# majidsina/rlmd

Hardware: NVIDIA B200
Metric: investor-steps/sec (leverage sweep) (higher is better)
Workload: dtype 2-bit codes, int32 counts, f64 log-wealth, f32 wealth

## Files before the change

include/rlmd_b200.h:

```cpp
#ifndef RLMD_B200_H
#define RLMD_B200_H

#include <stdint.h>

#ifdef __cplusplus
extern "C" {
#endif

#define B200_OK 0
#define B200_EINVAL (-1)
#define B200_ECUDA (-2)
#define B200_ELIMIT (-3)

#define B200_MAX_PEERS 8

const char* b200_last_error(void);
int b200_version(void);
int b200_device_info(int32_t* sm_count, int32_t* cc_major, int32_t* cc_minor);

enum {
  B200_LEV_DISCRETE = 0,
  B200_LEV_GBM = 1
};
enum {
// ... 13 lines not shown
  int64_t ld_outcomes;
  int64_t investor_offset;
  int64_t ld_out;
  uint64_t seed;
  int32_t horizon;
  int32_t n_grid;
  int32_t n_outcomes;
  int32_t kind;
  int32_t source;
  int32_t mode;
  float value_0;
  float log_mean;
  float sigma;
  int32_t variant;
  uint32_t thresholds[B200_MAX_OUTCOMES];
  int32_t outcome_bits;
  int32_t flags;
} b200_lev_desc;

#define B200_LEV_FLAG_FINAL_ONLY 1
#define B200_LEV_FLAG_STATE_OUT 2
#define B200_LEV_FLAG_BESIDE_SWEEP 4
#define B200_LEV_FLAG_RADIX_SELECT 8

int b200_lev_sweep(const b200_lev_desc* desc, const void* outcomes,
                   const float* factors_host, float* data_T, double* log_w,
                   int32_t* counts, void* stream);

int b200_lev_chunk(const b200_lev_desc* desc, const void* outcomes,
                   const float* factors_host, int32_t t_begin, int32_t t_end,
                   void* state, float* dump, void* stream);

int b200_lev_draw(const b200_lev_desc* desc, void* out, void* stream);

int b200_lev_from_counts(const b200_lev_desc* desc, const int32_t* counts,
                         const float* factors_host, float* data_T, double* log_w,
                         void* stream);

int b200_lev_pack(const uint8_t* codes, int64_t n_investors, int32_t horizon,
                  int64_t ld_codes, uint8_t* packed, int64_t ld_packed, void* stream);
int b200_lev_pack_bits(const uint8_t* codes, int64_t n_investors, int32_t horizon,
                       int64_t ld_codes, uint8_t* packed, int64_t ld_packed, int32_t bits,
                       void* stream);

typedef struct b200_tally_plan {
  int64_t rows_cap;
// ... 230 lines not shown
```

rlmd_b200/_lib.py:

```python
import ctypes as C
import os

_HERE = os.path.dirname(os.path.abspath(__file__))
LIB_PATH = os.path.join(_HERE, "librlmd_b200.so")

B200_OK, B200_EINVAL, B200_ECUDA, B200_ELIMIT = 0, -1, -2, -3
LEV_DISCRETE, LEV_GBM = 0, 1
SRC_STREAM, SRC_PHILOX = 0, 1
MODE_CHAIN, MODE_LOG = 1, 2
MAX_GRID, MAX_OUTCOMES = 64, 4


class LevDesc(C.Structure):
    _fields_ = [
        ("n_investors", C.c_int64),
        ("ld_outcomes", C.c_int64),
        ("investor_offset", C.c_int64),
        ("ld_out", C.c_int64),
        ("seed", C.c_uint64),
        ("horizon", C.c_int32),
        ("n_grid", C.c_int32),
        ("n_outcomes", C.c_int32),
        ("kind", C.c_int32),
        ("source", C.c_int32),
        ("mode", C.c_int32),
        ("value_0", C.c_float),
        ("log_mean", C.c_float),
        ("sigma", C.c_float),
        ("variant", C.c_int32),
        ("thresholds", C.c_uint32 * MAX_OUTCOMES),
        ("outcome_bits", C.c_int32),
        ("flags", C.c_int32),
    ]


LEV_FLAG_FINAL_ONLY, LEV_FLAG_STATE_OUT, LEV_FLAG_BESIDE_SWEEP, LEV_FLAG_RADIX_SELECT = 1, 2, 4, 8
MAX_PEERS = 8


class PeerSet(C.Structure):
    _fields_ = [
        ("workspace", C.c_void_p * MAX_PEERS),
        ("flags", C.c_void_p * MAX_PEERS),
        ("stage", C.c_void_p * MAX_PEERS),
        ("stage_rows", C.c_int64),
        ("world", C.c_int32),
        ("rank", C.c_int32),
        ("epoch", C.c_uint32),
        ("reserved", C.c_uint32),
    ]


class TallyPlan(C.Structure):
    _fields_ = [
        ("rows_cap", C.c_int64),
        ("bins_cap", C.c_int64),
        ("grid_cap", C.c_int32),
        ("world", C.c_int32),
    ]
# ... 219 lines not shown
```

rlmd_b200/csrc/common.cu:

```cuda
#include "common.cuh"

#include <cstring>

namespace b200 {

static thread_local char g_err[512] = "";

int set_error(int code, const char* fmt, ...) {
  va_list ap;
  va_start(ap, fmt);
  vsnprintf(g_err, sizeof(g_err), fmt, ap);
  va_end(ap);
  return code;
}

int check_cuda(cudaError_t e, const char* what) {
  if (e == cudaSuccess) return 0;
  return set_error(B200_ECUDA, "%s: %s", what, cudaGetErrorString(e));
}

int sm_count() {
  static int cached[64] = {0};
  int dev = 0;
  if (cudaGetDevice(&dev) != cudaSuccess || dev < 0 || dev >= 64) { cudaGetLastError(); return 148; }
  if (cached[dev] == 0) {
    int n = 0;
    if (cudaDeviceGetAttribute(&n, cudaDevAttrMultiProcessorCount, dev) != cudaSuccess || n <= 0) {
      cudaGetLastError();
      n = 148;
    }
    cached[dev] = n;
  }
  return cached[dev];
}

__global__ void __launch_bounds__(256)
exchange_pack_kernel(const long long* __restrict__ ws, int64_t words, int64_t rows, int64_t io, int64_t ic,
                     int64_t d_o, int64_t dc, double* __restrict__ staging) {
  const int64_t per = ic + dc, total = rows * per;
  for (int64_t i = (int64_t)blockIdx.x * blockDim.x + threadIdx.x; i < total; i += (int64_t)gridDim.x * blockDim.x) {
    const int64_t r = i / per, k = i - r * per;
// ... 61 lines not shown
```

rlmd_b200/csrc/common.cuh:

```cuda
#pragma once

#include <cuda_runtime.h>
#include <stdint.h>

#include <cstdarg>
#include <cstdio>

#include "../../include/rlmd_b200.h"

namespace b200 {

int set_error(int code, const char* fmt, ...);
int check_cuda(cudaError_t e, const char* what);

#define B200_CUDA(expr)                                   \
  do {                                                    \
    int _rc = ::b200::check_cuda((expr), #expr);          \
    if (_rc != 0) return _rc;                             \
  } while (0)

#define B200_REQUIRE(cond, ...)                                     \
  do {                                                              \
    if (!(cond)) return ::b200::set_error(B200_EINVAL, __VA_ARGS__); \
  } while (0)

int sm_count();

struct Philox4 {
  uint32_t x, y, z, w;
};

__host__ __device__ __forceinline__ uint32_t mulhi32(uint32_t a, uint32_t b) {
#ifdef __CUDA_ARCH__
  return __umulhi(a, b);
#else
  return (uint32_t)(((uint64_t)a * (uint64_t)b) >> 32);
#endif
}

__host__ __device__ __forceinline__ Philox4 philox4x32_10(uint32_t c0, uint32_t c1, uint32_t c2,
                                                           uint32_t c3, uint32_t k0, uint32_t k1) {
  const uint32_t M0 = 0xD2511F53u, M1 = 0xCD9E8D57u;
  const uint32_t W0 = 0x9E3779B9u, W1 = 0xBB67AE85u;
#pragma unroll
  for (int r = 0; r < 10; ++r) {
    uint32_t hi0 = mulhi32(M0, c0), lo0 = M0 * c0;
    uint32_t hi1 = mulhi32(M1, c2), lo1 = M1 * c2;
    uint32_t n0 = hi1 ^ c1 ^ k0;
    uint32_t n2 = hi0 ^ c3 ^ k1;
// ... 160 lines not shown
```

rlmd_b200/csrc/lev_sweep.cu:

```cuda
#include <cstdlib>

#include "lev_kernels.cuh"
#include "tally.cuh"

namespace b200 {

struct LogFactorTable {
  double lm[B200_MAX_OUTCOMES][B200_MAX_GRID];
};
struct LevGrid {
  float lev[B200_MAX_GRID];
};

static int64_t out_ld(const b200_lev_desc& d) { return d.ld_out > 0 ? d.ld_out : d.n_investors; }

template <int K>
__global__ void __launch_bounds__(128)
draw_discrete_kernel(const __grid_constant__ Thresholds th, uint64_t seed, int64_t investor_offset, int32_t H,
                     int64_t N, int64_t ld, uint8_t* __restrict__ out) {
  const int nblk = (H + 3) >> 2;
  const int64_t idx = (int64_t)blockIdx.x * blockDim.x + threadIdx.x;
  if (idx >= N * nblk) return;
  const int64_t row = idx / nblk;
  const int j = (int)(idx - row * nblk);
// ... 206 lines not shown
}

constexpr int PACKED_U = 6;

template <int BITS>
__device__ __forceinline__ uint32_t word_mask(int valid) {
  constexpr int PER = 32 / BITS;
  const int v = min(max(valid, 0), PER);
  return v >= PER ? 0xffffffffu : ((1u << (BITS * v)) - 1u);
}
template <int BITS>
__device__ __forceinline__ uint4 last_vector_mask(int valid) {
  constexpr int PER = 32 / BITS;
  return make_uint4(word_mask<BITS>(valid), word_mask<BITS>(valid - PER), word_mask<BITS>(valid - 2 * PER),
                    word_mask<BITS>(valid - 3 * PER));
}

template <int K, bool TALLY, int BITS = 2>
__global__ void __launch_bounds__(COUNT_WARPS * 32, 4)
log_discrete_packed_kernel(const uint8_t* __restrict__ outcomes, int64_t ldb, int32_t H, int64_t N, int32_t G,
                           const __grid_constant__ LogFactorTable lf, double logV0, float* __restrict__ data_T,
                           double* __restrict__ log_w, int32_t* __restrict__ counts, int64_t ldT, const TallyDev tally,
                           int32_t task_rows) {
  const int lane = threadIdx.x & 31;
  const int64_t warp_global = (int64_t)blockIdx.x * COUNT_WARPS + (threadIdx.x >> 5);
  const int64_t nwarps = (int64_t)gridDim.x * COUNT_WARPS;
  constexpr int PER_BYTE = 8 / BITS;
  const int nbytes = (H + PER_BYTE - 1) / PER_BYTE;
  const int full = H / PER_BYTE;
  const int nvec = (nbytes + 15) >> 4;
  const bool vec_rows = (ldb & 15) == 0 && ldb >= (int64_t)nvec * 16;
  const int iters = (nvec + 32 * PACKED_U - 1) / (32 * PACKED_U);
  const int rem = nvec - (iters - 1) * 32 * PACKED_U;
  const int tail_slots = (rem + 31) >> 5;
  const int tail_lanes = rem - (tail_slots - 1) * 32;
  const bool in_tail = lane < tail_lanes;
  const uint4 wm = lane == tail_lanes - 1 ? last_vector_mask<BITS>(H - (128 / BITS) * (nvec - 1))
                                          : make_uint4(~0u, ~0u, ~0u, ~0u);
  auto count_byte = [&](int t, uint32_t& s1, uint32_t& s2, uint32_t& s3, const uint8_t* __restrict__ p) {
    uint32_t c = p[t];
    if (t >= full) c &= (1u << (BITS * (H % PER_BYTE))) - 1u;
    if (BITS == 1) { s1 += __popc(c); return; }
    s1 += __popc(c & 0x55u);
    if (K >= 3) s2 += __popc((c >> 1) & 0x55u);
    if (K >= 4) s3 += __popc(c & (c >> 1) & 0x55u);
  };
// ... 36 lines not shown
        }
      } else {
        const uintptr_t addr = (uintptr_t)p;
        int head = (int)((16 - (addr & 15)) & 15);
        if (head > full) head = full;
        const int body = (full - head) >> 4;
        const int tail0 = head + (body << 4);
        for (int t = lane; t < head; t += 32) count_byte(t, s1, s2, s3, p);
        const uint4* __restrict__ q = reinterpret_cast<const uint4*>(p + head);
        for (int i = lane; i < body; i += 32) {
          const uint4 a = __ldcs(q + i);
          count_pair<K, BITS>(a.x, a.y, s1, s2, s3); count_pair<K, BITS>(a.z, a.w, s1, s2, s3);
        }
        for (int t = tail0 + lane; t < nbytes; t += 32) count_byte(t, s1, s2, s3, p);
      }
#pragma unroll
      for (int o = 16; o > 0; o >>= 1) {
        s1 += __shfl_xor_sync(0xffffffffu, s1, o);
        if (K >= 3) s2 += __shfl_xor_sync(0xffffffffu, s2, o);
        if (K >= 4) s3 += __shfl_xor_sync(0xffffffffu, s3, o);
      }
      if (lane == r) { m1 = s1; m2 = s2; m3 = s3; }
    }
    if (lane < nr) {
      const int64_t row = row0 + lane;
      int n[4];
      if (K == 2) { n[1] = (int)m1; n[0] = H - n[1]; n[2] = n[3] = 0; }
      else if (K == 3) { n[1] = (int)m1; n[2] = (int)m2; n[0] = H - n[1] - n[2]; n[3] = 0; }
      else { n[3] = (int)m3; n[1] = (int)(m1 - m3); n[2] = (int)(m2 - m3); n[0] = H - n[1] - n[2] - n[3]; }
      if (counts != nullptr) {
#pragma unroll
        for (int k = 0; k < K; ++k) counts[row * K + k] = n[k];
      }
      if (TALLY) {
        tally_insert(tally, tally_key(n[1], n[2], n[3]), 1u);
        continue;
      }
      double nd[K];
#pragma unroll
      for (int k = 0; k < K; ++k) nd[k] = (double)n[k];
      for (int g = 0; g < G; ++g) {
        double lw = logV0;
#pragma unroll
        for (int k = 0; k < K; ++k)
          if (n[k] > 0) lw += nd[k] * lf.lm[k][g];
        if (log_w != nullptr) log_w[(int64_t)g * ldT + row] = lw;
// ... 348 lines not shown
      }
      lf.lm[k][g] = v;
    }
  return 0;
}

static int run_log_discrete(const b200_lev_desc& d, const uint8_t* outcomes, const float* factors_host,
                            float* data_T, double* log_w, int32_t* counts, const TallyDev& tally, cudaStream_t st) {
  LogFactorTable lf;
  if (factors_host != nullptr) {
    if (int rc = make_log_table(d, factors_host, lf)) return rc;
  } else {
    memset(&lf, 0, sizeof(lf));
  }
  const double logV0 = log((double)d.value_0);
  const int64_t N = d.n_investors;
  static const int task_rows = [] { const char* e = getenv("B200_PACKED_TASK_ROWS"); int v = e ? atoi(e) : 32;
                                    return v < 1 ? 1 : v > 32 ? 32 : v; }();
  const bool packed = d.outcome_bits == 2 || d.outcome_bits == 1;
  const int64_t warps = packed ? (N + task_rows - 1) / task_rows : N;
  int64_t blocks = (warps + COUNT_WARPS - 1) / COUNT_WARPS;
  const int64_t cap = packed ? (int64_t)0x7fffffff : (int64_t)sm_count() * 8;
  if (blocks > cap) blocks = cap;
#define B200_LOG_LAUNCH(KERNEL, ...)                                                                                     \
  KERNEL<__VA_ARGS__><<<(unsigned)blocks, COUNT_WARPS * 32, 0, st>>>(outcomes, d.ld_outcomes, d.horizon, N, d.n_grid, lf, \
                                                                     logV0, data_T, log_w, counts, out_ld(d), tally B200_EXTRA)
  if (d.outcome_bits == 1) {
#define B200_EXTRA , task_rows
    if (tally.keys != nullptr) B200_LOG_LAUNCH(log_discrete_packed_kernel, 2, true, 1);
    else B200_LOG_LAUNCH(log_discrete_packed_kernel, 2, false, 1);
#undef B200_EXTRA
  } else if (d.outcome_bits == 2) {
#define B200_EXTRA , task_rows
    if (tally.keys != nullptr) {
      switch (d.n_outcomes) {
        case 2: B200_LOG_LAUNCH(log_discrete_packed_kernel, 2, true); break;
        case 3: B200_LOG_LAUNCH(log_discrete_packed_kernel, 3, true); break;
        default: B200_LOG_LAUNCH(log_discrete_packed_kernel, 4, true); break;
      }
    } else {
      switch (d.n_outcomes) {
        case 2: B200_LOG_LAUNCH(log_discrete_packed_kernel, 2, false); break;
        case 3: B200_LOG_LAUNCH(log_discrete_packed_kernel, 3, false); break;
        default: B200_LOG_LAUNCH(log_discrete_packed_kernel, 4, false); break;
      }
    }
#undef B200_EXTRA
#define B200_EXTRA
  } else {
    switch (d.n_outcomes) {
      case 2: B200_LOG_LAUNCH(log_discrete_stream_kernel, 2); break;
      case 3: B200_LOG_LAUNCH(log_discrete_stream_kernel, 3); break;
      default: B200_LOG_LAUNCH(log_discrete_stream_kernel, 4); break;
    }
  }
#undef B200_LOG_LAUNCH
#undef B200_EXTRA
  return check_cuda(cudaGetLastError(), "log_discrete_stream launch");
}

static int run_log_gbm(const b200_lev_desc& d, const float* x, const float* lev_host, float* data_T, double* log_w,
                       cudaStream_t st) {
  LevGrid lv;
  for (int g = 0; g < B200_MAX_GRID; ++g) lv.lev[g] = g < d.n_grid ? lev_host[g] : 0.f;
  const double logV0 = log((double)d.value_0);
  const int64_t N = d.n_investors;
  const bool saturate = (d.flags & B200_LEV_FLAG_FINAL_ONLY) == 0;
  const int64_t state_n = (d.flags & B200_LEV_FLAG_STATE_OUT) ? N : 0;
// ... 360 lines not shown
```

rlmd_b200/csrc/tally.cu:

```cuda
#include <cooperative_groups.h>

#include <algorithm>
#include <cstdlib>
#include <cstring>

#include "tally.cuh"

namespace b200 {

struct BinEntry {
  unsigned long long key, count;
};
static_assert(sizeof(BinEntry) == 16, "one 16-byte vector per bin");

constexpr int MERGE_CHUNK = 2048;
constexpr int EX_FLAG_BYTES = 128;

struct LogTable {
  double lm[B200_MAX_OUTCOMES][B200_MAX_GRID];
};

struct TallyLayout {
  long long* header;
  unsigned long long* keysA; uint32_t* countsA; uint64_t capA;
// ... 99 lines not shown
    const uint32_t m = __reduce_max_sync(0xffffffffu, b[q]);
    if ((threadIdx.x & 31) == 0 && m != 0u) atomicMax(s + q, m);
  }
  __syncthreads();
  if (threadIdx.x < 4 && s[threadIdx.x] != 0u)
    atomicMax(reinterpret_cast<unsigned long long*>(dst) + threadIdx.x, (unsigned long long)s[threadIdx.x]);
}

constexpr int COMPACT_PER = 8;
constexpr int COMPACT_CHUNK = 256 * COMPACT_PER;

template <bool MULTI>
__global__ void __launch_bounds__(256)
tally_compact_kernel(TallyDev t, unsigned long long* __restrict__ ukeys, uint32_t* __restrict__ ucnt,
                     int64_t out_cap, const __grid_constant__ PeerView P) {
  __shared__ BinEntry stage[COMPACT_CHUNK];
  __shared__ int n_s;
  __shared__ long long base_s;
  __shared__ uint32_t box_s[4];
  uint32_t box[4] = {0, 0, 0, 0};
  const uint64_t cap = t.mask + 1;
  const uint64_t base = (uint64_t)blockIdx.x * COMPACT_CHUNK;
  if (threadIdx.x == 0) n_s = 0;
  __syncthreads();
  unsigned long long key[COMPACT_PER];
  uint32_t cnt[COMPACT_PER];
#pragma unroll
  for (int u = 0; u < COMPACT_PER; ++u) {
    const uint64_t i = base + (uint64_t)u * 256 + threadIdx.x;
    key[u] = i < cap ? __ldcg(t.keys + i) : TALLY_EMPTY;
    cnt[u] = i < cap ? __ldcg(t.counts + i) : 0u;
  }
#pragma unroll
  for (int u = 0; u < COMPACT_PER; ++u) {
    if (key[u] == TALLY_EMPTY) continue;
    const uint64_t i = base + (uint64_t)u * 256 + threadIdx.x;
    t.keys[i] = TALLY_EMPTY;
    t.counts[i] = 0;
    if (!MULTI) box_add(box, key[u]);
    const int p = atomicAdd(&n_s, 1);
    stage[p].key = key[u];
    stage[p].count = cnt[u];
  }
  __syncthreads();
  const int n = n_s;
  if (!MULTI && n > 0) box_flush(box, t.header + TH_BOX_ACC, box_s);
// ... 311 lines not shown
    for (int q = 0; q < N; ++q) {
      const double x = lane < (int)(blockDim.x >> 5) ? scratch[q * 32 + lane] : 0.0;
      v[q] = warp_sum(x);
    }
  }
}

template <int NK>
__global__ void __launch_bounds__(SEL_THREADS)
tally_select_kernel(long long* __restrict__ header, const unsigned long long* __restrict__ ukeys,
                    const uint32_t* __restrict__ ucnt, float* __restrict__ wbuf, int64_t ldw, int32_t H,
                    const __grid_constant__ LogTable lf, double logV0, int64_t n_total, int64_t top,
                    double* __restrict__ stats, int32_t SEL_CACHE ,
                    int32_t force_radix) {
  namespace cg = cooperative_groups;
  cg::cluster_group cluster = cg::this_cluster();
  const int C = (int)cluster.num_blocks(), r = (int)cluster.block_rank();
  __shared__ SelShared sh;
  extern __shared__ __align__(16) uint8_t dyn[];
  float* cw = reinterpret_cast<float*>(dyn);
  uint32_t* cc = reinterpret_cast<uint32_t*>(dyn) + SEL_CACHE;
  uint16_t* cb = reinterpret_cast<uint16_t*>(cc + SEL_CACHE);
  SelShared* L = cluster.map_shared_rank(&sh, 0);

  const int g = blockIdx.x / C;
  const long long B = header[TH_NBINS];
  const long long n = n_total, K = top;
  const double qnan = __longlong_as_double(0x7ff8000000000000LL);
  double* s = stats + (int64_t)g * 12;
  if (header[TH_TIMEOUT] != 0 || header[TH_OVERFLOW] != 0) {
    if (r == 0 && threadIdx.x < 12) s[threadIdx.x] = qnan;
    return;
  }
  const int tid = threadIdx.x, lane = threadIdx.x & 31;
#ifdef B200_TALLY_DEBUG
  int stamp_i = 0;
#define STAMP() do { if (r == 0 && tid == 0 && (g == 0 || g == (int)(gridDim.x / C) - 1)) { header[TH_DEBUG + (g == 0 ? 0 : 24) + stamp_i++] = clock64(); } } while (0)
#else
#define STAMP() do {} while (0)
#endif
  STAMP();
  const long long per = (((B + C - 1) / C) + 3) & ~3LL;
  const long long lo = min(B, (long long)r * per), hi = min(B, lo + per);
  const int m = (int)(hi - lo);
  float* __restrict__ w = wbuf + (int64_t)g * ldw + lo;
  const uint32_t* __restrict__ cnt = ucnt + lo;
// ... 464 lines not shown
      d0 += sh.part_d[q][0]; d1 += sh.part_d[q][1]; d2 += sh.part_d[q][2];
      d3 += sh.part_d[q][3]; d4 += sh.part_d[q][4]; d5 += sh.part_d[q][5];
    }
    const double thr = (double)key_float(thr_key);
    const double dt = thr - mean_t, da = thr - mean_j;
    const double tt = (double)sh.res_i[6], ta = (double)sh.res_i[7];
    const double abs_top = d0 + (tt > 0 ? tt * fabs(dt) : 0.0);
    const double sq_top = d1 + (tt > 0 ? tt * dt * dt : 0.0);
    const double abs_adj = d2 + (ta > 0 ? ta * fabs(da) : 0.0);
    const double sq_adj = d3 + (ta > 0 ? ta * da * da : 0.0);
    s[0] = mean_a; s[1] = mean_t; s[2] = mean_j;
    s[3] = d4 / (double)n; s[4] = abs_top / (double)K; s[5] = abs_adj / (double)(n - K);
    s[6] = sqrt(d5 / (double)n); s[7] = sqrt(sq_top / (double)K); s[8] = sqrt(sq_adj / (double)(n - K));
    s[9] = (double)key_float(key_j[0]); s[10] = (double)key_float(key_j[2]); s[11] = (double)key_float(key_j[3]);
    const long long size[3] = {n, K, n - K};
    const double single[3] = {qnan, thr, (double)key_float(key_j[3])};
    for (int j = 0; j < 3; ++j) {
      if (sh.res_i[j]) { s[0 + j] = size[j] == 1 ? single[j] : qnan; s[3 + j] = qnan; s[6 + j] = qnan; }
      if (sh.res_i[3 + j]) s[9 + j] = qnan;
    }
  }
}

static void select_shape(int& cluster, int& cache) {
  static int c = [] {
    const char* e = getenv("B200_SELECT_CLUSTER");
    int x = e ? atoi(e) : 6;
    return x < 1 ? 1 : x > SEL_MAX_CLUSTER ? SEL_MAX_CLUSTER : x;
  }();
  static int k = [] {
    const char* e = getenv("B200_SELECT_CACHE");
    int x = e ? atoi(e) : 16384;
    return x < 0 ? 0 : x > 20480 ? 20480 : x;
  }();
  cluster = c;
  cache = k;
}

template <int K>
static int launch_select_k(int n_grid, long long* header, const unsigned long long* ukeys, const uint32_t* ucnt,
                           float* wbuf, int64_t ldw, int32_t H, const LogTable& lf, double logV0, int64_t n_total,
                           int64_t top, double* stats, bool beside_sweep, bool force_radix, cudaStream_t st) {
  static bool attr_set[64] = {false};
  int dev = 0;
  B200_CUDA(cudaGetDevice(&dev));
  int C = 1, cache = 0;
  select_shape(C, cache);
  static const bool forced = getenv("B200_SELECT_CLUSTER") != nullptr;
  if (beside_sweep && !forced) C = 2;
  const size_t dyn = (size_t)cache * 10;
  if (dev < 64 && !attr_set[dev]) {
    B200_CUDA(cudaFuncSetAttribute(tally_select_kernel<K>, cudaFuncAttributeMaxDynamicSharedMemorySize, (int)dyn));
    if (C > 8) B200_CUDA(cudaFuncSetAttribute(tally_select_kernel<K>, cudaFuncAttributeNonPortableClusterSizeAllowed, 1));
    attr_set[dev] = true;
  }
  cudaLaunchConfig_t cfg;
  memset(&cfg, 0, sizeof(cfg));
  cfg.gridDim = dim3((unsigned)(n_grid * C));
  cfg.blockDim = dim3(SEL_THREADS);
  cfg.dynamicSmemBytes = dyn;
  cfg.stream = st;
  cudaLaunchAttribute at[1];
  at[0].id = cudaLaunchAttributeClusterDimension;
  at[0].val.clusterDim.x = (unsigned)C;
  at[0].val.clusterDim.y = 1;
  at[0].val.clusterDim.z = 1;
  cfg.attrs = at;
  cfg.numAttrs = 1;
  return check_cuda(cudaLaunchKernelEx(&cfg, tally_select_kernel<K>, header, ukeys, ucnt, wbuf, ldw, H, lf, logV0,
                                       n_total, top, stats, (int32_t)cache, (int32_t)force_radix),
                    "tally_select launch");
}

static int grid_for(int64_t work, int threads, int per_sm) {
  const int64_t want = (work + threads - 1) / threads;
  const int64_t cap = (int64_t)sm_count() * per_sm;
  return (int)std::max<int64_t>(1, std::min(want, cap));
}

}

using namespace b200;

extern "C" int64_t b200_tally_workspace_bytes(const b200_tally_plan* plan) {
  if (plan_ok(plan)) return -1;
  return layout(*plan, nullptr).bytes;
}

extern "C" int64_t b200_tally_exchange_bytes(const b200_tally_plan* plan) {
  if (plan_ok(plan)) return -1;
  if (plan->world == 1) return 0;
// ... 6 lines not shown
  B200_REQUIRE(workspace != nullptr, "tally_reset: workspace is NULL");
  cudaStream_t st = (cudaStream_t)stream;
  const TallyLayout L = layout(*plan, workspace);
  B200_CUDA(cudaMemsetAsync(L.header, 0, TH_WORDS * 8, st));
  tally_clear_kernel<<<grid_for((int64_t)L.capA, 256, 8), 256, 0, st>>>(L.keysA, L.countsA, nullptr, nullptr, L.capA);
  if (plan->world > 1)
    tally_clear_kernel<<<grid_for((int64_t)L.capB, 256, 8), 256, 0, st>>>(L.keysB, nullptr, L.countsB, L.posB, L.capB);
  return check_cuda(cudaGetLastError(), "tally_reset launch");
}

extern "C" int b200_tally_finalize(const b200_tally_plan* plan, void* workspace, const b200_tally_peers* peers,
                                   int32_t phase, void* stream) {
  if (int rc = plan_ok(plan)) return rc;
  B200_REQUIRE(workspace != nullptr, "tally_finalize: workspace is NULL");
  B200_REQUIRE(phase >= -1 && phase <= 1, "tally_finalize: phase must be -1, 0 or 1");
  cudaStream_t st = (cudaStream_t)stream;
  const TallyLayout L = layout(*plan, workspace);
  TallyDev t{L.keysA, L.countsA, L.header, L.capA - 1};
  PeerView P;
  memset(&P, 0, sizeof(P));
  const int cgrid = (int)((L.capA + COMPACT_CHUNK - 1) / COMPACT_CHUNK);
  if (plan->world == 1) {
    if (phase == 1) return 0;
    tally_compact_kernel<false><<<cgrid, 256, 0, st>>>(t, L.ukeys, L.ucnt, std::min(plan->bins_cap, L.list_cap), P);
    return check_cuda(cudaGetLastError(), "tally_compact launch");
  }
  B200_REQUIRE(peers != nullptr, "tally_finalize: peers is NULL with world > 1");
  B200_REQUIRE(peers->world == plan->world && peers->rank >= 0 && peers->rank < peers->world,
               "tally_finalize: peers->world / rank do not fit the plan");
  B200_REQUIRE(peers->epoch >= 1, "tally_finalize: epoch starts at 1");
  const int64_t lbytes = (exchange_list_bytes(L.list_cap) + 255) & ~(int64_t)255;
  P.world = peers->world; P.rank = peers->rank; P.epoch = peers->epoch;
  for (int r = 0; r < peers->world; ++r) {
    B200_REQUIRE(peers->exchange[r] != nullptr, "tally_finalize: exchange buffer of rank %d is NULL", r);
    char* ex = (char*)peers->exchange[r];
    char* lst = ex + EX_FLAG_BYTES + (peers->epoch & 1) * lbytes;
    P.flags[r] = (uint32_t*)ex;
    P.list_count[r] = (long long*)lst;
    P.list[r] = (BinEntry*)(lst + 16);
  }
  if (phase != 1) {
    tally_compact_kernel<true><<<cgrid, 256, 0, st>>>(t, nullptr, nullptr, L.list_cap, P);
    B200_CUDA(cudaGetLastError());
  }
  if (phase == 0) return 0;
  const int64_t cat = (int64_t)plan->world * L.list_cap;
  tally_merge_kernel<<<sm_count() * 2, 256, 0, st>>>(P, L.header, L.concat, L.slot_of, L.keysB, L.countsB, L.posB,
                                                     L.capB, cat);
// ... 12 lines not shown
  B200_REQUIRE(workspace != nullptr && desc != nullptr && factors_host != nullptr && stats != nullptr,
               "tally_stats: NULL argument");
  B200_REQUIRE(desc->n_grid >= 1 && desc->n_grid <= plan->grid_cap, "tally_stats: n_grid must be in 1..grid_cap");
  B200_REQUIRE(desc->n_outcomes >= 2 && desc->n_outcomes <= B200_MAX_OUTCOMES, "tally_stats: n_outcomes out of range");
  B200_REQUIRE(desc->horizon >= 1 && desc->horizon <= TALLY_MAX_HORIZON, "tally_stats: horizon out of range");
  B200_REQUIRE(n_total >= 2 && n_total < ((int64_t)1 << 32), "tally_stats: need 2 <= n_total < 2^32");
  B200_REQUIRE(top >= 1 && top < n_total, "tally_stats: need 1 <= top < n_total (top=%lld)", (long long)top);
  cudaStream_t st = (cudaStream_t)stream;
  const TallyLayout L = layout(*plan, workspace);
  LogTable lf;
  for (int k = 0; k < B200_MAX_OUTCOMES; ++k)
    for (int g = 0; g < B200_MAX_GRID; ++g) {
      double v = 0.0;
      if (g < desc->n_grid && k < desc->n_outcomes) {
        const float m = factors_host[(int64_t)g * desc->n_outcomes + k];
        if (m < 0.0f) return set_error(B200_EINVAL, "tally_stats: factors must be >= 0 (m[%d][%d] = %g)", g, k, (double)m);
        v = log((double)m);
      }
      lf.lm[k][g] = v;
    }
  const double logV0 = log((double)desc->value_0);
  const bool beside = (desc->flags & B200_LEV_FLAG_BESIDE_SWEEP) != 0;
  const bool radix = (desc->flags & B200_LEV_FLAG_RADIX_SELECT) != 0;
  switch (desc->n_outcomes) {
    case 2: return launch_select_k<2>(desc->n_grid, L.header, L.ukeys, L.ucnt, L.wbuf, L.ldw, desc->horizon, lf, logV0, n_total, top, stats, beside, radix, st);
    case 3: return launch_select_k<3>(desc->n_grid, L.header, L.ukeys, L.ucnt, L.wbuf, L.ldw, desc->horizon, lf, logV0, n_total, top, stats, beside, radix, st);
    default: return launch_select_k<4>(desc->n_grid, L.header, L.ukeys, L.ucnt, L.wbuf, L.ldw, desc->horizon, lf, logV0, n_total, top, stats, beside, radix, st);
  }
}
```

rlmd_b200/engine.py:

```python
from __future__ import annotations

import ctypes as C
import math
import os
from typing import Optional, Sequence

import numpy as np
import torch

from . import _lib
from ._lib import BigBrainDesc, LevDesc, check, lib, ptr, require_cuda, stream_ptr

STAT_NAMES = (
    "mean", "mean_top", "mean_adj", "mad", "mad_top", "mad_adj",
    "std", "std_top", "std_adj", "med", "med_top", "med_adj",
)


def _round_up(x: int, m: int) -> int:
    return (x + m - 1) // m * m


def device_info() -> dict:
    require_cuda()
# ... 513 lines not shown
        self.kind, self.value_0, self.top = kind, float(value_0), int(top)
        self.factors = np.ascontiguousarray(factors, dtype=np.float32)
        self.group, self.n_total = group, n_total
        self.dev = _cuda_device(device)
        self.depth = max(1, int(depth)) if depth is not None else (2 if (group is not None or kind == "gbm") else 1)
        self.statistics = statistics or ("tally" if kind == "discrete" else "rows")
        if self.statistics not in ("tally", "rows") or (self.statistics == "tally" and kind != "discrete"):
            raise ValueError("statistics must be 'tally' (discrete gambles) or 'rows'")
        if self.statistics == "tally" and group is not None:
            from . import sharding

            if not sharding.peer_memory_available(group, self.dev):
                self.statistics = "rows"
        with torch.cuda.device(self.dev):
            self.sweep_stream = torch.cuda.Stream()
            self.stats_stream = torch.cuda.Stream(priority=-1) if self.depth > 1 else self.sweep_stream
        self.data_T = [None] * self.depth
        self.ws = [None] * self.depth
        self.tallies = [None] * self.depth
        self.free = [None] * self.depth
        self.count = 0
        self.last_sweep = None
        self.timing = False

    def submit(self, outcomes, factors: Optional[np.ndarray] = None) -> torch.Tensor:
        f = self.factors if factors is None else np.ascontiguousarray(factors, dtype=np.float32)
        g = f.shape[0]
        n, h = outcomes.shape
        b = self.count % self.depth
        self.count += 1
        tally = self.statistics == "tally"
        with torch.cuda.device(self.dev):
            cur = torch.cuda.current_stream()
            self.sweep_stream.wait_stream(cur)
            data = outcomes.data if isinstance(outcomes, PackedCodes) else outcomes
            data.record_stream(self.sweep_stream)
            with torch.cuda.stream(self.sweep_stream):
                if self.free[b] is not None:
                    self.sweep_stream.wait_event(self.free[b])
                if tally and (self.tallies[b] is None or self.tallies[b].plan.rows_cap < n):
                    from . import tally as _tally

                    self.tallies[b] = _tally.FinalTally(n, device=self.dev, group=self.group)
                if not tally and (self.data_T[b] is None or tuple(self.data_T[b].shape) != (g, n)):
                    self.data_T[b] = torch.empty((g, n), dtype=torch.float32, device=self.dev)
                    self.ws[b] = rowstats_workspace(g, self.dev)
                if self.timing:
                    t0 = torch.cuda.Event(enable_timing=True)
                    t0.record(self.sweep_stream)
                if tally:
                    self.tallies[b].add(outcomes, f.shape[1])
                else:
                    lev_sweep(self.kind, f, self.value_0, outcomes=outcomes, mode="log", out_data_T=self.data_T[b])
                swept = torch.cuda.Event(enable_timing=self.timing)
                swept.record(self.sweep_stream)
                if self.timing:
                    self.last_sweep = (t0, swept)
            n_total = self.n_total if self.n_total is not None else n
            with torch.cuda.stream(self.stats_stream):
                self.stats_stream.wait_event(swept)
                if tally:
                    self.tallies[b].finalize()
                    stats = self.tallies[b].stats(f, self.value_0, h, n_total=n_total, top=self.top,
                                                  beside_sweep=self.depth > 1)
                else:
                    stats = rowstats(self.data_T[b], self.top, n_total=self.n_total, group=self.group,
                                     workspace=self.ws[b])
                done = torch.cuda.Event()
                done.record(self.stats_stream)
                self.free[b] = done
                stats.record_stream(cur)
        return stats

    def submit_philox(self, n_investors: int, horizon: int, *, seed: int, investor_offset: int = 0,
                      log_mean: float, sigma: float, growth_quantiles: Optional[Sequence[float]] = (0.05, 0.5)):
        if self.kind != "gbm":
            raise ValueError("submit_philox is the GBM path")
        lev = self.factors.reshape(-1)
        g, n = lev.shape[0], int(n_investors)
        b = self.count % self.depth
        self.count += 1
        with torch.cuda.device(self.dev):
            cur = torch.cuda.current_stream()
            self.sweep_stream.wait_stream(cur)
            with torch.cuda.stream(self.sweep_stream):
                if self.free[b] is not None:
                    self.sweep_stream.wait_event(self.free[b])
                if self.data_T[b] is None or tuple(self.data_T[b].shape) != (g, n):
                    self.data_T[b] = torch.empty((g, n), dtype=torch.float32, device=self.dev)
                    self.ws[b] = rowstats_workspace(g, self.dev)
                if self.timing:
                    t0 = torch.cuda.Event(enable_timing=True)
                    t0.record(self.sweep_stream)
                res = lev_sweep("gbm", lev, self.value_0, n_investors=n, horizon=int(horizon), seed=seed,
                                investor_offset=investor_offset, log_mean=log_mean, sigma=sigma, mode="log",
# ... 1 lines not shown
                swept = torch.cuda.Event(enable_timing=self.timing)
                swept.record(self.sweep_stream)
                if self.timing:
                    self.last_sweep = (t0, swept)
            n_total = self.n_total if self.n_total is not None else n
            with torch.cuda.stream(self.stats_stream):
                self.stats_stream.wait_event(swept)
                stats = rowstats(self.data_T[b], self.top, n_total=n_total, group=self.group, workspace=self.ws[b])
                growth = None
                if growth_quantiles is not None:
                    res["state"].record_stream(self.stats_stream)
                    growth = gbm_growth_summary(res["state"], lev, int(horizon), self.value_0, data_T=self.data_T[b],
                                                quantiles=growth_quantiles, n_total=n_total, group=self.group)
                    growth.record_stream(cur)
                done = torch.cuda.Event()
                done.record(self.stats_stream)
                self.free[b] = done
                stats.record_stream(cur)
        return stats, growth

    def synchronize(self) -> None:
        self.sweep_stream.synchronize()
        self.stats_stream.synchronize()
        for t in self.tallies:
            if t is not None:
                t.check()
        if self.group is not None and self.statistics == "rows":
            from . import sharding

            sharding.raise_if_peers_timed_out(self.group, self.dev)


_FLT_MAX = 3.4028234663852886e38


def stats_to_reference_dtype(stats, n_total: int, top: int):
    sizes = (float(n_total), float(top), float(n_total - top))
    if isinstance(stats, torch.Tensor):
        out = stats.to(torch.float32)
        for j, m in enumerate(sizes):
            col = stats[..., 3 + j]
            out[..., 3 + j] = torch.where(col * m > _FLT_MAX, torch.full_like(out[..., 3 + j], float("inf")),
                                          out[..., 3 + j])
        return out
    st = np.asarray(stats, dtype=np.float64)
    with np.errstate(over="ignore"):
# ... 224 lines not shown
```

rlmd_b200/tally.py:

```python
from __future__ import annotations

import ctypes as C
from typing import Optional

import numpy as np
import torch

from . import _lib
from ._lib import LevDesc, TallyPeers, TallyPlan, check, lib, ptr, require_cuda, stream_ptr

_SRC_TYPES = {
    torch.uint8: _lib.DT_U8, torch.bool: _lib.DT_U8, torch.int32: _lib.DT_I32, torch.int64: _lib.DT_I64,
    torch.float32: _lib.DT_F32, torch.float64: _lib.DT_F64,
}

DEFAULT_BINS_CAP = 1 << 22


class TallyOverflow(RuntimeError):
    """More distinct count tuples than the plan's bins_cap: use lev_sweep + rowstats for this input."""


class TallyUnavailable(TallyOverflow):
    """The ranks of the group cannot map each other's memory (no peer access): the tally's exchange cannot be
# ... 54 lines not shown
            if world > 1:
                self.exchange = TallyExchange(lib.b200_tally_exchange_bytes(C.byref(self.plan)), group, self.dev)
            check(lib.b200_tally_reset(C.byref(self.plan), ptr(self.ws), stream_ptr()))
        self._staging = None
        self.rows = 0
        self.horizon = None

    def reset(self) -> None:
        with torch.cuda.device(self.dev):
            check(lib.b200_tally_reset(C.byref(self.plan), ptr(self.ws), stream_ptr()))
        self.rows = 0

    def _note(self, n: int, h: int) -> None:
        if self.horizon is not None and self.rows > 0 and self.horizon != h:
            raise ValueError("every row block of one sweep must have the same horizon")
        if self.rows + n > self.plan.rows_cap:
            raise ValueError(f"more than rows_cap = {self.plan.rows_cap} rows in one sweep")
        if h > _lib.TALLY_MAX_HORIZON:
            raise ValueError("the tally path needs horizon < 2^21")
        self.horizon = h
        self.rows += n

    def add(self, outcomes, n_outcomes: int, *, counts: Optional[torch.Tensor] = None,
            codes_out: Optional[torch.Tensor] = None) -> None:
        from .engine import PackedCodes

        k = int(n_outcomes)
        with torch.cuda.device(self.dev):
            if isinstance(outcomes, PackedCodes) or (outcomes.dtype == torch.uint8 and codes_out is None):
                packed = isinstance(outcomes, PackedCodes)
                data = outcomes.data if packed else outcomes
                n, h = outcomes.shape
                if not data.is_cuda or data.dim() != 2 or (n > 1 and data.stride(1) != 1):
                    raise ValueError("outcomes must be a [N,H] CUDA tensor with unit inner stride")
                self._note(n, h)
                d = LevDesc()
                d.kind, d.mode, d.source = _lib.LEV_DISCRETE, _lib.MODE_LOG, _lib.SRC_STREAM
                d.n_investors, d.horizon, d.n_grid, d.n_outcomes = n, h, 1, k
                d.value_0 = 1.0
                d.outcome_bits = outcomes.bits if packed else 8
                d.ld_outcomes = data.stride(0) if n > 1 else data.shape[1]
                check(lib.b200_lev_tally(C.byref(d), ptr(data), C.byref(self.plan), ptr(self.ws), ptr(counts),
                                         stream_ptr()))
                return
            t = outcomes
            if t.dtype not in _SRC_TYPES:
                raise TypeError(f"outcomes of dtype {t.dtype} are not an accepted format")
            if not t.is_cuda or t.dim() != 2 or (t.shape[0] > 1 and t.stride(1) != 1):
                raise ValueError("outcomes must be a [N,H] CUDA tensor with unit inner stride")
            n, h = t.shape
            self._note(n, h)
            ld = t.stride(0) if n > 1 else max(t.stride(0), h)
            ldc = 0
            if codes_out is not None:
                if codes_out.dtype != torch.uint8 or codes_out.shape[0] != n or codes_out.shape[1] < h:
                    raise ValueError("codes_out must be uint8 [N, >=H]")
                ldc = codes_out.stride(0) if n > 1 else codes_out.shape[1]
            check(lib.b200_lev_ingest(ptr(t), _SRC_TYPES[t.dtype], n, h, ld, k, ptr(codes_out), ldc, ptr(counts),
                                      C.byref(self.plan), ptr(self.ws), stream_ptr()))

    def add_host(self, host: torch.Tensor, n_outcomes: int, *, chunk_bytes: int = 256 << 20,
                 horizon: Optional[int] = None) -> int:
        from .engine import PackedCodes, _copy_stream

# ... 92 lines not shown
```

Baseline: 21990 billion.

## Chain tally sweep, compact and select kernels with programmatic dependent launch

Adds programmatic dependent launch (griddepcontrol) so that the packed tally sweep kernel, the compaction kernel and the select kernel can start their prologues before the previous kernel finishes. Each waits on griddepcontrol.wait before touching dependent data. With depth 1 it also drops the cross-stream events between the sweep and stats streams, and shrinks the default select cluster from 6 to 3 when early start is used. Timing stamps move to a separate stream, so the measured window now changes which work it covers, and the early-launched prologues add a correctness risk if they read data too soon.

```diff
diff --git a/include/rlmd_b200.h b/include/rlmd_b200.h
--- a/include/rlmd_b200.h
+++ b/include/rlmd_b200.h
@@ -59,6 +59,7 @@
 #define B200_LEV_FLAG_STATE_OUT 2
 #define B200_LEV_FLAG_BESIDE_SWEEP 4
 #define B200_LEV_FLAG_RADIX_SELECT 8
+#define B200_LEV_FLAG_EARLY_START 16
 
 int b200_lev_sweep(const b200_lev_desc* desc, const void* outcomes,
                    const float* factors_host, float* data_T, double* log_w,
diff --git a/rlmd_b200/_lib.py b/rlmd_b200/_lib.py
--- a/rlmd_b200/_lib.py
+++ b/rlmd_b200/_lib.py
@@ -34,7 +34,7 @@
     ]
 
 
-LEV_FLAG_FINAL_ONLY, LEV_FLAG_STATE_OUT, LEV_FLAG_BESIDE_SWEEP, LEV_FLAG_RADIX_SELECT = 1, 2, 4, 8
+LEV_FLAG_FINAL_ONLY, LEV_FLAG_STATE_OUT, LEV_FLAG_BESIDE_SWEEP, LEV_FLAG_RADIX_SELECT, LEV_FLAG_EARLY_START = 1, 2, 4, 8, 16
 MAX_PEERS = 8
 
 
diff --git a/rlmd_b200/csrc/common.cu b/rlmd_b200/csrc/common.cu
--- a/rlmd_b200/csrc/common.cu
+++ b/rlmd_b200/csrc/common.cu
@@ -1,5 +1,6 @@
 #include "common.cuh"
 
+#include <cstdlib>
 #include <cstring>
 
 namespace b200 {
@@ -17,6 +18,11 @@
 int check_cuda(cudaError_t e, const char* what) {
   if (e == cudaSuccess) return 0;
   return set_error(B200_ECUDA, "%s: %s", what, cudaGetErrorString(e));
+}
+
+bool pdl_enabled() {
+  static const bool on = [] { const char* e = getenv("B200_PDL"); return e == nullptr || atoi(e) != 0; }();
+  return on;
 }
 
 int sm_count() {
diff --git a/rlmd_b200/csrc/common.cuh b/rlmd_b200/csrc/common.cuh
--- a/rlmd_b200/csrc/common.cuh
+++ b/rlmd_b200/csrc/common.cuh
@@ -25,6 +25,14 @@
   } while (0)
 
 int sm_count();
+
+bool pdl_enabled();
+__device__ __forceinline__ void pdl_launch_dependents() { asm volatile("griddepcontrol.launch_dependents;" ::: "memory"); }
+__device__ __forceinline__ void pdl_wait() { asm volatile("griddepcontrol.wait;" ::: "memory"); }
+inline void set_pdl_attribute(cudaLaunchAttribute& a) {
+  a.id = cudaLaunchAttributeProgrammaticStreamSerialization;
+  a.val.programmaticStreamSerializationAllowed = 1;
+}
 
 struct Philox4 {
   uint32_t x, y, z, w;
diff --git a/rlmd_b200/csrc/lev_sweep.cu b/rlmd_b200/csrc/lev_sweep.cu
--- a/rlmd_b200/csrc/lev_sweep.cu
+++ b/rlmd_b200/csrc/lev_sweep.cu
@@ -252,6 +252,7 @@
                            const __grid_constant__ LogFactorTable lf, double logV0, float* __restrict__ data_T,
                            double* __restrict__ log_w, int32_t* __restrict__ counts, int64_t ldT, const TallyDev tally,
                            int32_t task_rows) {
+  if (TALLY) pdl_launch_dependents();
   const int lane = threadIdx.x & 31;
   const int64_t warp_global = (int64_t)blockIdx.x * COUNT_WARPS + (threadIdx.x >> 5);
   const int64_t nwarps = (int64_t)gridDim.x * COUNT_WARPS;
@@ -334,6 +335,7 @@
       }
       if (lane == r) { m1 = s1; m2 = s2; m3 = s3; }
     }
+    if (TALLY) pdl_wait();
     if (lane < nr) {
       const int64_t row = row0 + lane;
       int n[4];
@@ -728,28 +730,38 @@
   int64_t blocks = (warps + COUNT_WARPS - 1) / COUNT_WARPS;
   const int64_t cap = packed ? (int64_t)0x7fffffff : (int64_t)sm_count() * 8;
   if (blocks > cap) blocks = cap;
-#define B200_LOG_LAUNCH(KERNEL, ...)                                                                                     \
+  if (packed && tally.keys != nullptr) {
+    const auto kern = d.outcome_bits == 1 ? log_discrete_packed_kernel<2, true, 1>
+                      : d.n_outcomes == 2 ? log_discrete_packed_kernel<2, true>
+                      : d.n_outcomes == 3 ? log_discrete_packed_kernel<3, true>
+                                          : log_discrete_packed_kernel<4, true>;
+    B200_CUDA(cudaFuncSetAttribute(kern, cudaFuncAttributePreferredSharedMemoryCarveout, (int)cudaSharedmemCarveoutMaxL1));
+    cudaLaunchConfig_t cfg;
+    memset(&cfg, 0, sizeof(cfg));
+    cfg.gridDim = dim3((unsigned)blocks);
+    cfg.blockDim = dim3(COUNT_WARPS * 32);
+    cfg.stream = st;
+    cudaLaunchAttribute at[1];
+    set_pdl_attribute(at[0]);
+    cfg.attrs = at;
+    cfg.numAttrs = (d.flags & B200_LEV_FLAG_EARLY_START) != 0 && pdl_enabled() ? 1 : 0;
+    return check_cuda(cudaLaunchKernelEx(&cfg, kern, outcomes, d.ld_outcomes, d.horizon, N, d.n_grid, lf, logV0, data_T,
+                                         log_w, counts, out_ld(d), tally, (int32_t)task_rows),
+                      "log_discrete_packed (tally) launch");
+  }
+#define B200_LOG_LAUNCH(KERNEL, ...)                                                                                  \
   KERNEL<__VA_ARGS__><<<(unsigned)blocks, COUNT_WARPS * 32, 0, st>>>(outcomes, d.ld_outcomes, d.horizon, N, d.n_grid, lf, \
                                                                      logV0, data_T, log_w, counts, out_ld(d), tally B200_EXTRA)
   if (d.outcome_bits == 1) {
 #define B200_EXTRA , task_rows
-    if (tally.keys != nullptr) B200_LOG_LAUNCH(log_discrete_packed_kernel, 2, true, 1);
-    else B200_LOG_LAUNCH(log_discrete_packed_kernel, 2, false, 1);
+    B200_LOG_LAUNCH(log_discrete_packed_kernel, 2, false, 1);
 #undef B200_EXTRA
   } else if (d.outcome_bits == 2) {
 #define B200_EXTRA , task_rows
-    if (tally.keys != nullptr) {
-      switch (d.n_outcomes) {
-        case 2: B200_LOG_LAUNCH(log_discrete_packed_kernel, 2, true); break;
-        case 3: B200_LOG_LAUNCH(log_discrete_packed_kernel, 3, true); break;
-        default: B200_LOG_LAUNCH(log_discrete_packed_kernel, 4, true); break;
-      }
-    } else {
-      switch (d.n_outcomes) {
-        case 2: B200_LOG_LAUNCH(log_discrete_packed_kernel, 2, false); break;
-        case 3: B200_LOG_LAUNCH(log_discrete_packed_kernel, 3, false); break;
-        default: B200_LOG_LAUNCH(log_discrete_packed_kernel, 4, false); break;
-      }
+    switch (d.n_outcomes) {
+      case 2: B200_LOG_LAUNCH(log_discrete_packed_kernel, 2, false); break;
+      case 3: B200_LOG_LAUNCH(log_discrete_packed_kernel, 3, false); break;
+      default: B200_LOG_LAUNCH(log_discrete_packed_kernel, 4, false); break;
     }
 #undef B200_EXTRA
 #define B200_EXTRA
diff --git a/rlmd_b200/csrc/tally.cu b/rlmd_b200/csrc/tally.cu
--- a/rlmd_b200/csrc/tally.cu
+++ b/rlmd_b200/csrc/tally.cu
@@ -145,6 +145,8 @@
   const uint64_t cap = t.mask + 1;
   const uint64_t base = (uint64_t)blockIdx.x * COMPACT_CHUNK;
   if (threadIdx.x == 0) n_s = 0;
+  pdl_launch_dependents();
+  pdl_wait();
   __syncthreads();
   unsigned long long key[COMPACT_PER];
   uint32_t cnt[COMPACT_PER];
@@ -502,6 +504,8 @@
   uint32_t* cc = reinterpret_cast<uint32_t*>(dyn) + SEL_CACHE;
   uint16_t* cb = reinterpret_cast<uint16_t*>(cc + SEL_CACHE);
   SelShared* L = cluster.map_shared_rank(&sh, 0);
+  pdl_launch_dependents();
+  pdl_wait();
 
   const int g = blockIdx.x / C;
   const long long B = header[TH_NBINS];
@@ -1012,10 +1016,11 @@
   }
 }
 
-static void select_shape(int& cluster, int& cache) {
+static void select_shape(int& cluster, int& cache, bool early) {
   static int c = [] {
     const char* e = getenv("B200_SELECT_CLUSTER");
-    int x = e ? atoi(e) : 6;
+    if (e == nullptr) return 0;
+    const int x = atoi(e);
     return x < 1 ? 1 : x > SEL_MAX_CLUSTER ? SEL_MAX_CLUSTER : x;
   }();
   static int k = [] {
@@ -1023,19 +1028,20 @@
     int x = e ? atoi(e) : 16384;
     return x < 0 ? 0 : x > 20480 ? 20480 : x;
   }();
-  cluster = c;
+  cluster = c != 0 ? c : early ? 3 : 6;
   cache = k;
 }
 
 template <int K>
 static int launch_select_k(int n_grid, long long* header, const unsigned long long* ukeys, const uint32_t* ucnt,
                            float* wbuf, int64_t ldw, int32_t H, const LogTable& lf, double logV0, int64_t n_total,
-                           int64_t top, double* stats, bool beside_sweep, bool force_radix, cudaStream_t st) {
+                           int64_t top, double* stats, bool beside_sweep, bool force_radix, bool early,
+                           cudaStream_t st) {
   static bool attr_set[64] = {false};
   int dev = 0;
   B200_CUDA(cudaGetDevice(&dev));
   int C = 1, cache = 0;
-  select_shape(C, cache);
+  select_shape(C, cache, early);
   static const bool forced = getenv("B200_SELECT_CLUSTER") != nullptr;
   if (beside_sweep && !forced) C = 2;
   const size_t dyn = (size_t)cache * 10;
@@ -1050,13 +1056,14 @@
   cfg.blockDim = dim3(SEL_THREADS);
   cfg.dynamicSmemBytes = dyn;
   cfg.stream = st;
-  cudaLaunchAttribute at[1];
+  cudaLaunchAttribute at[2];
   at[0].id = cudaLaunchAttributeClusterDimension;
   at[0].val.clusterDim.x = (unsigned)C;
   at[0].val.clusterDim.y = 1;
   at[0].val.clusterDim.z = 1;
+  set_pdl_attribute(at[1]);
   cfg.attrs = at;
-  cfg.numAttrs = 1;
+  cfg.numAttrs = early ? 2 : 1;
   return check_cuda(cudaLaunchKernelEx(&cfg, tally_select_kernel<K>, header, ukeys, ucnt, wbuf, ldw, H, lf, logV0,
                                        n_total, top, stats, (int32_t)cache, (int32_t)force_radix),
                     "tally_select launch");
@@ -1109,8 +1116,18 @@
   const int cgrid = (int)((L.capA + COMPACT_CHUNK - 1) / COMPACT_CHUNK);
   if (plan->world == 1) {
     if (phase == 1) return 0;
-    tally_compact_kernel<false><<<cgrid, 256, 0, st>>>(t, L.ukeys, L.ucnt, std::min(plan->bins_cap, L.list_cap), P);
-    return check_cuda(cudaGetLastError(), "tally_compact launch");
+    cudaLaunchConfig_t cfg;
+    memset(&cfg, 0, sizeof(cfg));
+    cfg.gridDim = dim3((unsigned)cgrid);
+    cfg.blockDim = dim3(256);
+    cfg.stream = st;
+    cudaLaunchAttribute at[1];
+    set_pdl_attribute(at[0]);
+    cfg.attrs = at;
+    cfg.numAttrs = pdl_enabled() ? 1 : 0;
+    return check_cuda(cudaLaunchKernelEx(&cfg, tally_compact_kernel<false>, t, L.ukeys, L.ucnt,
+                                         (int64_t)std::min(plan->bins_cap, L.list_cap), P),
+                      "tally_compact launch");
   }
   B200_REQUIRE(peers != nullptr, "tally_finalize: peers is NULL with world > 1");
   B200_REQUIRE(peers->world == plan->world && peers->rank >= 0 && peers->rank < peers->world,
@@ -1169,9 +1186,10 @@
   const double logV0 = log((double)desc->value_0);
   const bool beside = (desc->flags & B200_LEV_FLAG_BESIDE_SWEEP) != 0;
   const bool radix = (desc->flags & B200_LEV_FLAG_RADIX_SELECT) != 0;
+  const bool early = plan->world == 1 && !beside && pdl_enabled();
   switch (desc->n_outcomes) {
-    case 2: return launch_select_k<2>(desc->n_grid, L.header, L.ukeys, L.ucnt, L.wbuf, L.ldw, desc->horizon, lf, logV0, n_total, top, stats, beside, radix, st);
-    case 3: return launch_select_k<3>(desc->n_grid, L.header, L.ukeys, L.ucnt, L.wbuf, L.ldw, desc->horizon, lf, logV0, n_total, top, stats, beside, radix, st);
-    default: return launch_select_k<4>(desc->n_grid, L.header, L.ukeys, L.ucnt, L.wbuf, L.ldw, desc->horizon, lf, logV0, n_total, top, stats, beside, radix, st);
-  }
-}
+    case 2: return launch_select_k<2>(desc->n_grid, L.header, L.ukeys, L.ucnt, L.wbuf, L.ldw, desc->horizon, lf, logV0, n_total, top, stats, beside, radix, early, st);
+    case 3: return launch_select_k<3>(desc->n_grid, L.header, L.ukeys, L.ucnt, L.wbuf, L.ldw, desc->horizon, lf, logV0, n_total, top, stats, beside, radix, early, st);
+    default: return launch_select_k<4>(desc->n_grid, L.header, L.ukeys, L.ucnt, L.wbuf, L.ldw, desc->horizon, lf, logV0, n_total, top, stats, beside, radix, early, st);
+  }
+}
diff --git a/rlmd_b200/engine.py b/rlmd_b200/engine.py
--- a/rlmd_b200/engine.py
+++ b/rlmd_b200/engine.py
@@ -559,6 +559,8 @@
         self.count = 0
         self.last_sweep = None
         self.timing = False
+        self._timing_stream = None
+        self._sweep_opens = None
 
     def submit(self, outcomes, factors: Optional[np.ndarray] = None) -> torch.Tensor:
         f = self.factors if factors is None else np.ascontiguousarray(factors, dtype=np.float32)
@@ -567,6 +569,9 @@
         b = self.count % self.depth
         self.count += 1
         tally = self.statistics == "tally"
+        chain = tally and self.depth == 1
+        if not (self.timing and chain):
+            self._sweep_opens = None
         with torch.cuda.device(self.dev):
             cur = torch.cuda.current_stream()
             self.sweep_stream.wait_stream(cur)
@@ -583,31 +588,44 @@
                     self.data_T[b] = torch.empty((g, n), dtype=torch.float32, device=self.dev)
                     self.ws[b] = rowstats_workspace(g, self.dev)
                 if self.timing:
-                    t0 = torch.cuda.Event(enable_timing=True)
-                    t0.record(self.sweep_stream)
+                    t0 = self._sweep_opens if chain and self._sweep_opens is not None else self._stamp()
                 if tally:
-                    self.tallies[b].add(outcomes, f.shape[1])
+                    self.tallies[b].add(outcomes, f.shape[1], early_start=chain)
                 else:
                     lev_sweep(self.kind, f, self.value_0, outcomes=outcomes, mode="log", out_data_T=self.data_T[b])
-                swept = torch.cuda.Event(enable_timing=self.timing)
-                swept.record(self.sweep_stream)
                 if self.timing:
-                    self.last_sweep = (t0, swept)
+                    self.last_sweep = (t0, self._stamp())
             n_total = self.n_total if self.n_total is not None else n
             with torch.cuda.stream(self.stats_stream):
-                self.stats_stream.wait_event(swept)
+                if self.depth > 1:
+                    swept = torch.cuda.Event()
+                    swept.record(self.sweep_stream)
+                    self.stats_stream.wait_event(swept)
                 if tally:
                     self.tallies[b].finalize()
+                    if self.timing and chain:
+                        self._sweep_opens = self._stamp()
                     stats = self.tallies[b].stats(f, self.value_0, h, n_total=n_total, top=self.top,
                                                   beside_sweep=self.depth > 1)
                 else:
                     stats = rowstats(self.data_T[b], self.top, n_total=self.n_total, group=self.group,
                                      workspace=self.ws[b])
-                done = torch.cuda.Event()
-                done.record(self.stats_stream)
-                self.free[b] = done
+                if self.depth > 1:
+                    done = torch.cuda.Event()
+                    done.record(self.stats_stream)
+                    self.free[b] = done
                 stats.record_stream(cur)
         return stats
+
+    def _stamp(self) -> torch.cuda.Event:
+        if self._timing_stream is None:
+            self._timing_stream = torch.cuda.Stream(self.dev)
+        mark = torch.cuda.Event()
+        mark.record(self.sweep_stream)
+        self._timing_stream.wait_event(mark)
+        ev = torch.cuda.Event(enable_timing=True)
+        ev.record(self._timing_stream)
+        return ev
 
     def submit_philox(self, n_investors: int, horizon: int, *, seed: int, investor_offset: int = 0,
                       log_mean: float, sigma: float, growth_quantiles: Optional[Sequence[float]] = (0.05, 0.5)):
@@ -655,6 +673,8 @@
     def synchronize(self) -> None:
         self.sweep_stream.synchronize()
         self.stats_stream.synchronize()
+        if self._timing_stream is not None:
+            self._timing_stream.synchronize()
         for t in self.tallies:
             if t is not None:
                 t.check()
diff --git a/rlmd_b200/tally.py b/rlmd_b200/tally.py
--- a/rlmd_b200/tally.py
+++ b/rlmd_b200/tally.py
@@ -100,7 +100,7 @@
         self.rows += n
 
     def add(self, outcomes, n_outcomes: int, *, counts: Optional[torch.Tensor] = None,
-            codes_out: Optional[torch.Tensor] = None) -> None:
+            codes_out: Optional[torch.Tensor] = None, early_start: bool = False) -> None:
         from .engine import PackedCodes
 
         k = int(n_outcomes)
@@ -118,6 +118,7 @@
                 d.value_0 = 1.0
                 d.outcome_bits = outcomes.bits if packed else 8
                 d.ld_outcomes = data.stride(0) if n > 1 else data.shape[1]
+                d.flags = _lib.LEV_FLAG_EARLY_START if early_start else 0
                 check(lib.b200_lev_tally(C.byref(d), ptr(data), C.byref(self.plan), ptr(self.ws), ptr(counts),
                                          stream_ptr()))
                 return
```

New measurement: 23210 billion, median of 6. 1.06x the previous value.
